# Bebra777228/PolGen-RVC

Hardware: AMD Instinct MI355X
Metric: real-time-factor (audio-sec/wall-sec) per GPU, 30s@16kHz RMVPE->48kHz (higher is better)
Workload: dtype f32 (conv products as 3 fp16 MFMAs of a hi/lo split, fp32 accumulate; fp32 elsewhere)

## Files before the change

### polgen-rvc_amd/csrc/api.hip

```cpp
#include "api_internal.h"

using namespace rvcx;
using namespace rvcx::api;

bool rvcx::api::localize_overflow(Ctx& c) {
  WeightRegion* best_r = nullptr;
  int best = 0, best_i = -1;
  for (WeightRegion* r : all_regions(c, nullptr)) {
    int i = -1;
    const int v = r->first_overflow(&i);
    if (v > best) {
      best = v;
      best_i = i;
      best_r = r;
    }
  }
  if (!best_r) return false;
  best_r->drop_flag(best_i);
  return true;
}

void rvcx::api::reset_after_failure(Ctx& c) {
  (void)hipDeviceSynchronize();
  c.arena.reset();
  c.arena_f0.reset();
  c.arena_hub.reset();
}

bool rvcx::api::debug_hooks_enabled() {
  static const bool on = [] {
    const char* e = getenv("RVCX_DEBUG");
    return e && atoi(e) != 0;
  }();
  return on;
}

std::vector<WeightRegion*> rvcx::api::all_regions(Ctx& c, uint64_t* hash) {
  std::vector<WeightRegion*> r;
  uint64_t h = 1469598103934665603ull;
  auto add = [&](WeightRegion* w, uint64_t tag) {
    h = (h ^ tag) * 1099511628211ull;
    h = (h ^ (w ? w->layout_hash() : 0)) * 1099511628211ull;
    if (w) r.push_back(w);
  };
  add(c.hubert ? c.hubert->region.get() : nullptr, 1);
  add(c.rmvpe ? c.rmvpe->region.get() : nullptr, 2);
  add(c.fcpe ? c.fcpe->region.get() : nullptr, 4);
  add(c.crepe ? c.crepe->region.get() : nullptr, 5);
  for (size_t i = 0; i < c.synths.size(); ++i) add(c.synths[i] ? c.synths[i]->region.get() : nullptr, 16 + i);
  add(c.index ? c.index->region.get() : nullptr, 3);
  if (hash) *hash = h;
  return r;
// ... 254 lines not shown
          dev_ptrs[k] = r->chunk_base(i);
          nbytes[k] = (int64_t)r->chunk_used(i);
        }
    return k;
  } catch (const std::exception& e) {
    g_last_error = e.what();
    if (C) C->last_error = e.what();
    return -1;
  }
}

int rvcx_weights_clone(rvcx_ctx* ctx, rvcx_ctx* src) {
  CtxLock ga, gb;
  if (ctx && src && ctx != src) {
    ga = CtxLock(ctx->mu, std::defer_lock);
    gb = CtxLock(src->mu, std::defer_lock);
    std::lock(ga, gb);
  }
  API_BEGIN_ONCE(ctx)
  if (!src) fail("weights_clone: null source context");
  if (src->c.device != C->device) fail("weights_clone: contexts live on different devices (use the RCCL broadcast)");
  uint64_t ha = 0, hb = 0;
  std::vector<WeightRegion*> ra = all_regions(src->c, &ha), rb = all_regions(*C, &hb);
  if (ha != hb || ra.size() != rb.size()) fail("weights_clone: the two contexts hold different model layouts");
  RVCX_HIP(hipDeviceSynchronize());
  for (size_t r = 0; r < ra.size(); ++r) {
    if (ra[r]->n_chunks() != rb[r]->n_chunks()) fail("weights_clone: chunk lists differ");
    for (int i = 0; i < ra[r]->n_chunks(); ++i) {
      if (ra[r]->chunk_used(i) != rb[r]->chunk_used(i)) fail("weights_clone: chunk sizes differ");
      RVCX_HIP(hipMemcpy(rb[r]->chunk_base(i), ra[r]->chunk_base(i), ra[r]->chunk_used(i), hipMemcpyDeviceToDevice));
    }
    rb[r]->adopt();
  }
  API_END
}

int rvcx_weights_adopt(rvcx_ctx* ctx) {
  API_BEGIN_ONCE(ctx)
  RVCX_HIP(hipDeviceSynchronize());
  for (WeightRegion* r : all_regions(*C, nullptr)) r->adopt();
  API_END
}

int rvcx_load_rmvpe(rvcx_ctx* ctx, const rvcx_rmvpe_cfg* cfg, const rvcx_tensor* tbl, int n) {
  API_BEGIN_ONCE(ctx)
  TensorTable t = make_table(tbl, n);
  C->rmvpe = rmvpe_load(*C, *cfg, t);
  (void)bigru_probe_publish();
  API_END
}

int rvcx_load_crepe(rvcx_ctx* ctx, const rvcx_tensor* tbl, int n) {
  API_BEGIN_ONCE(ctx)
  TensorTable t = make_table(tbl, n);
  C->crepe = crepe_load(*C, t);
  API_END
}

int rvcx_load_fcpe(rvcx_ctx* ctx, const rvcx_fcpe_cfg* cfg, const rvcx_tensor* tbl, int n) {
  API_BEGIN_ONCE(ctx)
  TensorTable t = make_table(tbl, n);
  C->fcpe = fcpe_load(*C, *cfg, t);
  API_END
}

int rvcx_load_hubert(rvcx_ctx* ctx, const rvcx_hubert_cfg* cfg, const rvcx_tensor* tbl, int n) {
  API_BEGIN_ONCE(ctx)
  TensorTable t = make_table(tbl, n);
  C->hubert = hubert_load(*C, *cfg, t);
  API_END
}

int rvcx_load_index(rvcx_ctx* ctx, const float* big_npy, int64_t n, int dim) {
// ... 66 lines not shown
```

### polgen-rvc_amd/csrc/api_internal.h

```cpp
#pragma once
#include "../../include/rvcx.h"

#include <atomic>
#include <cmath>
#include <cstdlib>
#include <deque>
#include <mutex>
#include <unordered_map>

#include "ctx.h"
#include "effects.h"
#include "layers.h"
#include "models.h"
#include "ops.h"
#include "pipeline.h"

namespace rvcx {
namespace api {

struct Ticket {
  rvcx_ticket id = 0;
  enum State { InFlight, Done, Failed } state = InFlight;
  std::string error;
  int model_id = 0;
// ... 84 lines not shown
  std::unordered_map<int, std::unique_ptr<rvcx::api::StreamSession>> sessions;
  int next_session = 1;
  std::recursive_mutex mu;
  std::deque<rvcx::api::TicketPtr> inflight;
  std::unordered_map<rvcx_ticket, rvcx::api::TicketPtr> tickets;
  std::deque<std::pair<rvcx_ticket, float>> leads;
  int fx_passes[3] = {0, 0, 0};
  int fx_groups = 0;
  rvcx::Arena load_arena;
};
namespace rvcx {
namespace api {

using CtxLock = std::unique_lock<std::recursive_mutex>;
inline CtxLock lock_ctx(rvcx_ctx* h) { return h ? CtxLock(h->mu) : CtxLock(); }

inline thread_local std::string g_last_error;

struct Fp32Scope {
  bool saved;
  explicit Fp32Scope(bool on) : saved(g_force_fp32) { g_force_fp32 = saved || on; }
  ~Fp32Scope() { g_force_fp32 = saved; }
};
struct GruScope {
  bool saved;
  explicit GruScope(bool on) : saved(g_gru_no_cluster) { g_gru_no_cluster = saved || on; }
  ~GruScope() { g_gru_no_cluster = saved; }
};
constexpr int kMaxAttempts = 6;

std::vector<WeightRegion*> all_regions(Ctx& c, uint64_t* hash);
bool localize_overflow(Ctx& c);
void reset_after_failure(Ctx& c);
void drain_tickets(rvcx_ctx* h);

template <typename F>
void run_attempts(Ctx* C, bool repeat, bool gru_plain, F&& body) {
  {
    const int last = repeat ? kMaxAttempts - 1 : 0;
    for (int attempt = 0; attempt <= last; ++attempt) {
      Fp32Scope fp32_scope(attempt > 0 && attempt == last);
      GruScope gru_scope(gru_plain);
      C->launch_seq = 0;
      C->err_snapshot = false;
      try {
        body(C);
      } catch (const GruTimeout&) {
        if (!repeat || gru_plain) throw;
        gru_plain = true;
        C->gru_fallbacks++;
        reset_after_failure(*C);
        --attempt;
        continue;
      }
      if (attempt < last && C->take_overflow()) {
        C->fp32_reruns++;
        if (!localize_overflow(*C)) attempt = last - 1;
        continue;
      }
      if (attempt > 0 && attempt == last) (void)C->take_overflow();
      break;
    }
  }
}

template <typename F>
int api_call(rvcx_ctx* ctxp, bool repeat, F&& body, bool drain = true) {
  Ctx* C = ctxp ? &ctxp->c : nullptr;
  CtxLock guard = lock_ctx(ctxp);
  try {
    if (!C) fail("null context");
    RVCX_HIP(hipSetDevice(C->device));
    if (drain) drain_tickets(ctxp);
    if (!repeat) C->arena_budget = 0;
    run_attempts(C, repeat, false, body);
    return 0;
  } catch (const std::exception& e) {
    g_last_error = e.what();
    if (C) {
      C->last_error = e.what();
      reset_after_failure(*C);
    }
    (void)hipGetLastError();
    return -1;
  }
}

StreamSession& get_session(rvcx_ctx* h, int id);

// ... 35 lines not shown
```

### polgen-rvc_amd/csrc/api_ops.hip

```cpp
#include "api_internal.h"
#include "h3_device.h"

using namespace rvcx;
using namespace rvcx::api;

static void to_host(Ctx& c, float* h, const float* d, size_t n) {
  RVCX_HIP(hipMemcpyAsync(h, d, n * sizeof(float), hipMemcpyDeviceToHost, c.stream));
  RVCX_HIP(hipStreamSynchronize(c.stream));
}
#define TEMP_REGION(C) WeightRegion tmp_region_; RegionScope tmp_scope_(*(C), tmp_region_)

extern "C" {

int rvcx_op_conv1d(rvcx_ctx* ctx, const float* x, const float* w, const float* bias, const float* res,
                   float* y, int B, int Cin, int Tin, int Cout, int K, int stride, int dil,
                   int pad_left, int Tout, int groups, int pre_lrelu, float pre_slope, int act,
                   float act_slope, const int32_t* lens_in, const int32_t* lens_out) {
  API_BEGIN(ctx)
  TEMP_REGION(C);
  size_t nx = (size_t)B * Cin * Tin, ny = (size_t)B * Cout * Tout;
  C->arena.reserve((nx + 2 * ny) * 4 + (64 << 20));
  C->arena.reset();
  ConvW L = make_conv(*C, w, bias, Cout, Cin / groups, K, groups, true);
  float* dx = to_dev(*C, x, nx);
// ... 596 lines not shown
    to_host(*C, stats, dst, (size_t)B * Cc * 2);
    std::vector<uint16_t> raw(n * 2);
    RVCX_HIP(hipMemcpy(raw.data(), ds, raw.size() * 2, hipMemcpyDeviceToHost));
    decode_split_cf(raw, B, Cc, T, y_split);
  }
  C->arena.reset();
  API_END
}

int rvcx_op_hubert_conv0(rvcx_ctx* ctx, const float* wav, const float* w, const float* gamma, const float* beta, int B, int Cc,
                         int n, int K, int stride, float eps, const int32_t* lens, int fused, float* stats, float* y_split,
                         uint16_t* raw_split) {
  API_BEGIN(ctx)
  TEMP_REGION(C);
  if (!wav || !w || !gamma || !beta || !stats || !y_split || B <= 0 || Cc <= 0 || K <= 0 || stride <= 0 || n < K)
    fail("op_hubert_conv0: bad argument");
  const int T0 = (n - K) / stride + 1;
  if (lens)
    for (int b = 0; b < B; ++b)
      if (lens[b] < 1 || lens[b] > T0) fail("op_hubert_conv0: lens outside [1, T0]");
  const size_t ny = (size_t)B * Cc * T0;
  C->arena.reserve(((size_t)B * n + 2 * ny + (size_t)B * Cc * 2) * 4 + (64 << 20));
  C->arena.reset();
  hipStream_t s = C->stream;
  ConvW L = make_conv(*C, w, nullptr, Cc, 1, K, 1);
  float* dw = to_dev(*C, wav, (size_t)B * n);
  const float *dg = to_dev(*C, gamma, Cc), *db = to_dev(*C, beta, Cc);
  const int* dl = (lens ? to_dev(*C, lens, B) : nullptr);
  float* dst = C->arena.alloc<float>((size_t)B * Cc * 2);
  float* ds = C->arena.alloc<float>(ny);
  RVCX_HIP(hipMemsetAsync(dst, 0xff, (size_t)B * Cc * 8, s));
  RVCX_HIP(hipMemsetAsync(ds, 0xff, ny * 4, s));
  if (fused) {
    launch_hubert_conv0_gn_gelu_split(dw, (long)n, L.w, K, stride, L.cin_gp * L.cout_gp, dg, db, nullptr, dst, ds, B, Cc, T0, eps,
                                      s, dl, C->dev_err, nullptr, 0);
  } else {
    float* dm = C->arena.alloc<float>(ny);
    RVCX_HIP(hipMemsetAsync(dm, 0xff, ny * 4, s));
    ConvArgs a = conv1d_args(L, dw, dm, B, n, T0, stride, 1, 0);
    a.lens_out = dl;
    C->conv(a);
    launch_groupnorm_gelu_split(dm, dg, db, dst, ds, B, Cc, T0, eps, s, dl, C->dev_err, nullptr, 0);
  }
  RVCX_HIP(hipGetLastError());
  to_host(*C, stats, dst, (size_t)B * Cc * 2);
  std::vector<uint16_t> raw(ny * 2);
  RVCX_HIP(hipMemcpy(raw.data(), ds, raw.size() * 2, hipMemcpyDeviceToHost));
  decode_split_cf(raw, B, Cc, T0, y_split);
  if (raw_split) std::memcpy(raw_split, raw.data(), raw.size() * 2);
  C->arena.reset();
  API_END
}

int rvcx_op_sine_source(rvcx_ctx* ctx, const float* f0, const float* noise, const float* lin_wb, int B, int T, int upp, float sr,
                        const int32_t* lens, float* har) {
  API_BEGIN(ctx)
  if (!f0 || !noise || !lin_wb || !har || B <= 0 || T <= 0 || upp <= 0) fail("op_sine_source: bad argument");
  const size_t n = (size_t)B * T * upp;
  C->arena.reserve(n * 8 + (size_t)B * T * 24 + (64 << 20));
  C->arena.reset();
  hipStream_t s = C->stream;
  const float* df = to_dev(*C, f0, (size_t)B * T);
  const float* dn = to_dev(*C, noise, n);
  const float* dwb = to_dev(*C, lin_wb, 2);
  const int* dl = (lens ? to_dev(*C, lens, B) : nullptr);
  double* sc = C->arena.alloc<double>((size_t)B * T * 2);
  float* dh = C->arena.alloc<float>(n);
// ... 238 lines not shown
```

### polgen-rvc_amd/csrc/hubert.hip

```cpp
#include <cmath>

#include "models.h"
#include "ops.h"

namespace rvcx {

std::unique_ptr<HubertModel> hubert_load(Ctx& c, const rvcx_hubert_cfg& cfg, const TensorTable& t) {
  auto M = std::make_unique<HubertModel>();
  RegionScope scope(c, *M->region);
  M->cfg = cfg;
  const int E = cfg.embed_dim;
  for (int i = 0; i < cfg.n_conv; ++i) {
    const std::string p = "feature_extractor.conv_layers." + std::to_string(i) + ".0.weight";
    auto w = t.f32(p);
    const auto shp = t.shape(p);
    RVCX_CHECK((int)shp[2] == cfg.conv_kernels[i], "hubert conv kernel mismatch");
    M->convs.push_back(make_conv(c, w.data(), nullptr, (int)shp[0], (int)shp[1], (int)shp[2], 1));
  }
  M->gn_g = c.slab.upload(t.f32("feature_extractor.conv_layers.0.2.weight"));
  M->gn_b = c.slab.upload(t.f32("feature_extractor.conv_layers.0.2.bias"));
  M->ln0_g = c.slab.upload(t.f32("layer_norm.weight"));
  M->ln0_b = c.slab.upload(t.f32("layer_norm.bias"));
  {
    auto w = t.f32("post_extract_proj.weight");
// ... 100 lines not shown
  int64_t Tin = n;
  const float* x = wav;
  float* y = bufa;
  static const bool no_split = getenv("RVCX_NO_SPLIT") && atoi(getenv("RVCX_NO_SPLIT")) != 0;
  std::vector<ConvArgs> la(cf.n_conv);
  {
    int64_t ti = n;
    for (int i = 0; i < cf.n_conv; ++i) {
      const int64_t to = (ti - cf.conv_kernels[i]) / cf.conv_strides[i] + 1;
      RVCX_CHECK(to > 0, "hubert: input too short");
      la[i] = conv1d_args(m.convs[i], nullptr, nullptr, B, (int)ti, (int)to, cf.conv_strides[i], 1, 0);
      if (i > 0) la[i].act = ACT_GELU;
      ti = to;
    }
  }
  auto split_after = [&](int i) {
    if (no_split || i + 1 >= cf.n_conv || i > 3 || cf.conv_strides[i + 1] != 2 || !conv_h3_split_ok(la[i + 1])) return false;
    return i == 0 ? C % 16 == 0 : (cf.conv_kernels[i + 1] == cf.conv_kernels[i] && conv_h3_split_ok(la[i]));
  };
  for (int i = 0; i < cf.n_conv; ++i) {
    const int64_t Tout = la[i].Nout;
    ConvArgs a = la[i];
    a.x = x;
    a.y = y;
    if (i == 0 && wav_bs > 0) a.x_bs = wav_bs;
    a.lens_out = d_tl[i];
    if (i > 0 && split_after(i - 1)) a.x_split = x;
    if (i > 0 && split_after(i)) {
      a.y_split = y;
      a.y = nullptr;
    }
    static const bool fuse0_on = !getenv("RVCX_HUBERT_FUSE0") || atoi(getenv("RVCX_HUBERT_FUSE0")) != 0;
    const bool fuse0 = i == 0 && fuse0_on && split_after(0) && m.convs[0].cin == 1 && m.convs[0].groups == 1 && !m.convs[0].bias &&
                       m.convs[0].w && cf.conv_kernels[0] <= 16 && (long)B * (C / 16) >= 256;
    if (fuse0) {
      float* z = (y == bufa) ? bufb : bufa;
      double* part = A.alloc<double>(hubert_conv0_part_doubles(B, C, (int)Tout));
      launch_hubert_conv0_gn_gelu_split(wav, wav_bs > 0 ? wav_bs : (long)n, m.convs[0].w, cf.conv_kernels[0], cf.conv_strides[0],
                                        m.convs[0].cin_gp * m.convs[0].cout_gp, m.gn_g, m.gn_b, part, gn_stats, z, B, C, (int)Tout, 1e-5f, s, d_t0,
                                        c.dev_err, m.convs[1].ovf_word, ++c.launch_seq);
      c.flops += 2.0 * cf.conv_kernels[0] * C * (double)Tout * B * 2;
      RVCX_HIP(hipGetLastError());
      y = z;
      x = y;
      y = (y == bufa) ? bufb : bufa;
      Tin = Tout;
      continue;
    }
    c.conv_on(a, s);
    if (i == 0) {
      float* z = (y == bufa) ? bufb : bufa;
      if (split_after(0))
        launch_groupnorm_gelu_split(y, m.gn_g, m.gn_b, gn_stats, z, B, C, (int)Tout, 1e-5f, s, d_t0, c.dev_err,
                                    m.convs[1].ovf_word, ++c.launch_seq);
      else
        launch_groupnorm_gelu(y, m.gn_g, m.gn_b, z, B, C, (int)Tout, 1e-5f, s, d_t0);
      y = z;
    }
    x = y;
    y = (y == bufa) ? bufb : bufa;
    Tin = Tout;
  }
  const int T = (int)Tin;
  if (after_extractor) (*after_extractor)();
  float* ln = y;
  launch_layernorm_c(x, m.ln0_g, m.ln0_b, ln, B, C, T, 1e-5f, nullptr, s);
  float* h = A.alloc<float>((size_t)B * E * T);
// ... 137 lines not shown
```

### polgen-rvc_amd/csrc/models.h

```cpp
#pragma once
#include <functional>

#include "../../include/rvcx.h"
#include "ctx.h"
#include "layers.h"

namespace rvcx {

struct SynthModel {
  std::shared_ptr<WeightRegion> region = std::make_shared<WeightRegion>();
  rvcx_synth_cfg cfg{};
  int upp = 1;
  int dec_rf_frames = 0;
  ConvW emb_phone;
  const float* emb_pitch = nullptr;
  struct EncLayer {
    ConvW qkv, o, ffn1, ffn2;
    AttFlag att;
    const float *rel_k = nullptr, *rel_v = nullptr;
    const float *g1 = nullptr, *b1 = nullptr, *g2 = nullptr, *b2 = nullptr;
  };
  std::vector<EncLayer> enc;
  ConvW proj;
  struct Flow {
    ConvW pre, post, cond, in_l[3], rs_l[3];
  };
  Flow flows[4];
  ConvW conv_pre, cond, conv_post;
  const float* lin_wb = nullptr;
  struct Stage {
    ConvT1dW up;
    ConvW noise;
    int noise_stride = 1, noise_pad = 0;
    ConvW noise_dense;
    int noise_dense_cin = 0;
    int ch = 0;
    ConvW c1[4][3], c2[4][3];
  };
  std::vector<Stage> stages;
  const float* emb_g = nullptr;
};

std::unique_ptr<SynthModel> synth_load(Ctx& c, const rvcx_synth_cfg& cfg, const TensorTable& t);

struct SynthIO {
  int B = 1, T = 0;
  const int* lens_host = nullptr;
  const float* phone_ct = nullptr;
  const int* pitch = nullptr;
  const float* pitchf = nullptr;
  const int* sid_host = nullptr;
  const float* z_noise = nullptr;
  const float* src_noise = nullptr;
  float* out = nullptr;
  int dec_skip = 0;
  int skip_head = 0;
  float* stats_out = nullptr;
  float* z_out = nullptr;
  hipEvent_t ev_decoder = nullptr;
};
size_t synth_arena_bytes(const SynthModel& m, int B, int T);
void synth_forward(Ctx& c, const SynthModel& m, const SynthIO& io, hipEvent_t* stage_ev );

struct RmvpeModel {
  std::shared_ptr<WeightRegion> region = std::make_shared<WeightRegion>();
  rvcx_rmvpe_cfg cfg{};
  ConvW stft;
  ConvW melfb;
  const float* bn0 = nullptr;
  struct Block {
    ConvW c1, c2, sc;
    bool has_sc = false;
    int cin = 0, cout = 0;
// ... 131 lines not shown
```

### polgen-rvc_amd/csrc/ops.hip

```cpp
#include <algorithm>
#include <cmath>
#include <vector>

#include "conv.h"
#include "h3_device.h"
#include "ops.h"

namespace rvcx {

__device__ __forceinline__ float wave_sum(float v) {
#pragma unroll
  for (int o = 32; o > 0; o >>= 1) v += __shfl_xor(v, o);
  return v;
}

__device__ __forceinline__ float gelu_erf(float v) {
  return 0.5f * v * (1.f + erff(v * 0.70710678118654752440f));
}

constexpr int LN_TX = 16, LN_PARTS = 16, LN_MAXC = 1024, LN_RPT = LN_MAXC / LN_PARTS;
__global__ __launch_bounds__(256) void layernorm_c_kernel(const float* __restrict__ x,
                                                          const float* __restrict__ gamma,
                                                          const float* __restrict__ beta, float* __restrict__ y,
                                                          int C, int T, float eps, const int* lens) {
// ... 221 lines not shown
  for (t = T + tid; t < Trow; t += 512) yr[t] = 0.f;
}

__global__ __launch_bounds__(256) void groupnorm_gelu_split_kernel(const float* __restrict__ x, const float* __restrict__ stats,
                                                                   const float* __restrict__ gamma,
                                                                   const float* __restrict__ beta, void* __restrict__ ys, int C,
                                                                   int Trow, const int* __restrict__ lens, int* ovf,
                                                                   int* ovf_layer, int seq) {
  const int t = blockIdx.x * 256 + threadIdx.x, cg = blockIdx.y, b = blockIdx.z;
  if (t >= Trow) return;
  const int T = lens ? lens[b] : Trow;
  const float* xr = x + ((long)b * C + cg * 8) * Trow + t;
  half8 hi, lo;
#pragma unroll
  for (int q = 0; q < 8; ++q) {
    const int c = cg * 8 + q;
    const float mean = stats[((long)b * C + c) * 2], rstd = stats[((long)b * C + c) * 2 + 1];
    float v = gelu_erf((xr[(long)q * Trow] - mean) * rstd * gamma[c] + beta[c]);
    v = t < T ? v : 0.f;
    if (!(fabsf(v) < kH3ActLimit)) {
      if (ovf) atomicOr(ovf, kErrH3Overflow);
      if (ovf_layer) atomicMax(ovf_layer, 0x7fffffff - seq);
    }
    const _Float16 vh = (_Float16)v;
    hi[q] = vh;
    lo[q] = (_Float16)((v - (float)vh) * kH3Scale);
  }
  uint4* base = reinterpret_cast<uint4*>(static_cast<char*>(ys) + (long)b * C * Trow * 4);
  const int chunk = cg >> 1, hh = cg & 1;
  base[(long)((chunk * 2 + 0) * 2 + hh) * Trow + t] = __builtin_bit_cast(uint4, hi);
  base[(long)((chunk * 2 + 1) * 2 + hh) * Trow + t] = __builtin_bit_cast(uint4, lo);
}

template <int CB>
__global__ __launch_bounds__(512) void hubert_conv0_stats_kernel(const float* __restrict__ wav, long wav_bs,
                                                                 const float* __restrict__ w, int K, int stride, int Cp, int C,
                                                                 int Trow, const int* __restrict__ lens, float* __restrict__ stats,
                                                                 float eps) {
  __shared__ float ws[16 * CB];
  __shared__ double red[2][8][CB];
  const int c0 = blockIdx.x * CB, b = blockIdx.y;
  const int T = lens ? lens[b] : Trow;
  for (int idx = threadIdx.x; idx < K * CB; idx += 512) ws[idx] = w[(long)(idx / CB) * Cp + c0 + (idx % CB)];
  __syncthreads();
  const float* xb = wav + (long)b * wav_bs;
  const int tid = threadIdx.x, lane = tid & 63, wave = tid >> 6;
  double s[CB], q[CB];
#pragma unroll
  for (int j = 0; j < CB; ++j) s[j] = q[j] = 0.0;
  auto fir = [&](int t, float (&acc)[CB]) {
#pragma unroll
    for (int j = 0; j < CB; ++j) acc[j] = 0.f;
    const float* xp = xb + (long)t * stride;
    for (int kk = 0; kk < K; ++kk) {
      const float xv = xp[kk];
#pragma unroll
      for (int j = 0; j < CB; ++j) acc[j] = fmaf(ws[kk * CB + j], xv, acc[j]);
    }
  };
  int t = tid;
  for (; t + 3 * 512 < T; t += 4 * 512) {
    float v0[CB], v1[CB], v2[CB], v3[CB];
    fir(t, v0);
    fir(t + 512, v1);
    fir(t + 1024, v2);
    fir(t + 1536, v3);
#pragma unroll
    for (int j = 0; j < CB; ++j) {
      s[j] += ((double)v0[j] + (double)v1[j]) + ((double)v2[j] + (double)v3[j]);
      q[j] += ((double)v0[j] * v0[j] + (double)v1[j] * v1[j]) + ((double)v2[j] * v2[j] + (double)v3[j] * v3[j]);
    }
  }
  for (; t < T; t += 512) {
    float v[CB];
    fir(t, v);
#pragma unroll
    for (int j = 0; j < CB; ++j) {
      s[j] += v[j];
      q[j] += (double)v[j] * v[j];
    }
  }
#pragma unroll
  for (int j = 0; j < CB; ++j) {
#pragma unroll
    for (int d = 32; d > 0; d >>= 1) {
      s[j] += __shfl_xor(s[j], d, 64);
      q[j] += __shfl_xor(q[j], d, 64);
    }
    if (lane == 0) {
      red[0][wave][j] = s[j];
      red[1][wave][j] = q[j];
    }
  }
  __syncthreads();
  if (tid < CB && c0 + tid < C) {
    double ts = 0.0, tq = 0.0;
#pragma unroll
    for (int wv = 0; wv < 8; ++wv) {
      ts += red[0][wv][tid];
      tq += red[1][wv][tid];
    }
    const double meand = ts / T;
    const float mean = (float)meand;
    const float var = (float)fmax(tq / T - meand * meand, 0.0);
    const float rstd = 1.f / sqrtf(var + eps);
    stats[((long)b * C + c0 + tid) * 2] = mean;
    stats[((long)b * C + c0 + tid) * 2 + 1] = rstd;
  }
}

__global__ __launch_bounds__(256) void hubert_conv0_apply_kernel(const float* __restrict__ wav, long wav_bs,
                                                                 const float* __restrict__ w, int K, int stride, int Cp,
                                                                 const float* __restrict__ stats, const float* __restrict__ gamma,
                                                                 const float* __restrict__ beta, void* __restrict__ ys, int C,
                                                                 int Trow, const int* __restrict__ lens, int* ovf, int* ovf_layer,
                                                                 int seq) {
  __shared__ float ws[16 * 8];
  const int cg = blockIdx.y, b = blockIdx.z;
  for (int idx = threadIdx.x; idx < K * 8; idx += 256) ws[idx] = w[(long)(idx >> 3) * Cp + cg * 8 + (idx & 7)];
  __syncthreads();
  const int t = blockIdx.x * 256 + threadIdx.x;
  if (t >= Trow) return;
  const int T = lens ? lens[b] : Trow;
  float acc[8];
#pragma unroll
  for (int qq = 0; qq < 8; ++qq) acc[qq] = 0.f;
  if (t < T) {
    const float* xb = wav + (long)b * wav_bs + (long)t * stride;
    for (int kk = 0; kk < K; ++kk) {
      const float xv = xb[kk];
#pragma unroll
      for (int qq = 0; qq < 8; ++qq) acc[qq] = fmaf(ws[kk * 8 + qq], xv, acc[qq]);
    }
  }
  half8 hi, lo;
#pragma unroll
  for (int qq = 0; qq < 8; ++qq) {
    const int c = cg * 8 + qq;
    const float mean = stats[((long)b * C + c) * 2], rstd = stats[((long)b * C + c) * 2 + 1];
    float v = gelu_erf((acc[qq] - mean) * rstd * gamma[c] + beta[c]);
    v = t < T ? v : 0.f;
    if (!(fabsf(v) < kH3ActLimit)) {
      if (ovf) atomicOr(ovf, kErrH3Overflow);
      if (ovf_layer) atomicMax(ovf_layer, 0x7fffffff - seq);
    }
    const _Float16 vh = (_Float16)v;
    hi[qq] = vh;
    lo[qq] = (_Float16)((v - (float)vh) * kH3Scale);
  }
  uint4* base = reinterpret_cast<uint4*>(static_cast<char*>(ys) + (long)b * C * Trow * 4);
  const int chunk = cg >> 1, hh = cg & 1;
  base[(long)((chunk * 2 + 0) * 2 + hh) * Trow + t] = __builtin_bit_cast(uint4, hi);
  base[(long)((chunk * 2 + 1) * 2 + hh) * Trow + t] = __builtin_bit_cast(uint4, lo);
}

size_t hubert_conv0_part_doubles(int, int, int) { return 0; }

void launch_hubert_conv0_gn_gelu_split(const float* wav, long wav_bs, const float* w, int K, int stride, int Cp, const float* gamma,
                                       const float* beta, double* part, float* stats, void* y_split, int B, int C, int T,
                                       float eps, hipStream_t s, const int* lens, int* ovf, int* ovf_layer, int seq) {
  RVCX_CHECK(C % 16 == 0 && K <= 16, "hubert conv0 fusion: channels must be a multiple of 16, at most 16 taps");
  (void)part;
  if ((long)B * (C / 16) >= 256)
    hipLaunchKernelGGL(hubert_conv0_stats_kernel<16>, dim3(C / 16, B), dim3(512), 0, s, wav, wav_bs, w, K, stride, Cp, C, T, lens,
                       stats, eps);
  else
    hipLaunchKernelGGL(hubert_conv0_stats_kernel<4>, dim3(C / 4, B), dim3(512), 0, s, wav, wav_bs, w, K, stride, Cp, C, T, lens,
                       stats, eps);
  hipLaunchKernelGGL(hubert_conv0_apply_kernel, dim3(cdiv(T, 256), C / 8, B), dim3(256), 0, s, wav, wav_bs, w, K, stride, Cp,
                     stats, gamma, beta, y_split, C, T, lens, ovf, ovf_layer, seq);
}

void launch_groupnorm_gelu(const float* x, const float* gamma, const float* beta, float* y, int B, int C, int T,
                           float eps, hipStream_t s, const int* lens) {
  hipLaunchKernelGGL(groupnorm_gelu_kernel<false>, dim3(C, B), dim3(512), 0, s, x, gamma, beta, y, C, T, eps, lens);
}

void launch_groupnorm_gelu_split(const float* x, const float* gamma, const float* beta, float* stats, void* y_split, int B,
                                 int C, int T, float eps, hipStream_t s, const int* lens, int* ovf, int* ovf_layer, int seq) {
  RVCX_CHECK(C % 16 == 0, "groupnorm_gelu_split: channels must be a multiple of 16");
  hipLaunchKernelGGL(groupnorm_gelu_kernel<true>, dim3(C, B), dim3(512), 0, s, x, gamma, beta, stats, C, T, eps, lens);
  hipLaunchKernelGGL(groupnorm_gelu_split_kernel, dim3(cdiv(T, 256), C / 8, B), dim3(256), 0, s, x, stats, gamma, beta,
                     y_split, C, T, lens, ovf, ovf_layer, seq);
}

__global__ void transpose_kernel(const float* __restrict__ x, float* __restrict__ y, int R, int Cc) {
  __shared__ float tile[32][33];
  const int b = blockIdx.z;
  const float* xb = x + (long)b * R * Cc;
  float* yb = y + (long)b * R * Cc;
  int c = blockIdx.x * 32 + threadIdx.x;
  for (int j = threadIdx.y; j < 32; j += 8) {
    int r = blockIdx.y * 32 + j;
    if (r < R && c < Cc) tile[j][threadIdx.x] = xb[(long)r * Cc + c];
  }
  __syncthreads();
  int r2 = blockIdx.y * 32 + threadIdx.x;
  for (int j = threadIdx.y; j < 32; j += 8) {
    int c2 = blockIdx.x * 32 + j;
    if (r2 < R && c2 < Cc) yb[(long)c2 * R + r2] = tile[threadIdx.x][j];
  }
// ... 556 lines not shown
```

### polgen-rvc_amd/csrc/synth.hip

```cpp
#include <algorithm>
#include <cmath>
#include <cstdlib>

#include "models.h"
#include "ops.h"

namespace rvcx {

std::vector<float> wn_weight(const TensorTable& t, const std::string& p, int dim) {
  if (t.has(p + ".weight")) return t.f32(p + ".weight");
  std::string gn = p + ".parametrizations.weight.original0", vn = p + ".parametrizations.weight.original1";
  if (!t.has(gn)) {
    gn = p + ".weight_g";
    vn = p + ".weight_v";
  }
  std::vector<float> g = t.f32(gn), v = t.f32(vn);
  const auto shp = t.shape(vn);
  RVCX_CHECK(shp.size() == 3, "weight-norm tensor must be 3-D: " + p);
  const int64_t d0 = shp[0], d1 = shp[1], d2 = shp[2];
  std::vector<float> w(v.size());
  if (dim == 0) {
    RVCX_CHECK((int64_t)g.size() == d0, "weight_g shape: " + p);
    for (int64_t a = 0; a < d0; ++a) {
      double ss = 0.0;
// ... 91 lines not shown
    std::vector<float> b = t.f32(p + ".bias");
    S.up = make_convT1d(c, w.data(), b.data(), ch, co, k, u, (k - u) / 2);
    int sf0 = 1;
    for (int j = i + 1; j < cfg.n_ups; ++j) sf0 *= cfg.up_rates[j];
    S.noise = load_conv(c, t, "dec.noise_convs." + std::to_string(i));
    S.noise_stride = sf0;
    S.noise_pad = sf0 > 1 ? sf0 / 2 : 0;
    if (sf0 >= 16 && S.noise.k == 2 * sf0 && S.noise.cin == 1) {
      const std::vector<float> w1 = t.f32("dec.noise_convs." + std::to_string(i) + ".weight");
      const std::vector<float> b1 = t.f32("dec.noise_convs." + std::to_string(i) + ".bias");
      const int sp = (sf0 + 15) / 16 * 16, kn = 2 * sf0, half = sf0 / 2;
      std::vector<float> w2((size_t)co * sp * 3, 0.f);
      for (int o = 0; o < co; ++o)
        for (int c2 = 0; c2 < sf0; ++c2)
          for (int m2 = 0; m2 < 3; ++m2) {
            const int j = sf0 * (m2 - 1) + c2 + half;
            if (j >= 0 && j < kn) w2[((size_t)o * sp + c2) * 3 + m2] = w1[(size_t)o * kn + j];
          }
      S.noise_dense = make_conv(c, w2.data(), b1.data(), co, sp, 3, 1, true);
      S.noise_dense_cin = sp;
    }
    S.ch = co;
    for (int j = 0; j < cfg.n_resblocks; ++j)
      for (int m = 0; m < 3; ++m) {
        const std::string rp = "dec.resblocks." + std::to_string(i * cfg.n_resblocks + j);
        S.c1[j][m] = load_conv(c, t, rp + ".convs1." + std::to_string(m), true, true, true);
        S.c2[j][m] = load_conv(c, t, rp + ".convs2." + std::to_string(m), true, true, true);
      }
    M->stages.push_back(S);
    ch = co;
  }
  M->emb_g = c.slab.upload(t.f32("emb_g.weight"));
  {
    double rf = 3.0, rate = 1.0;
    for (int i = 0; i < cfg.n_ups; ++i) {
      rf += ((cfg.up_kernels[i] - 1) / cfg.up_rates[i] + 1) / rate;
      rate *= cfg.up_rates[i];
      int res = 0;
      for (int j = 0; j < cfg.n_resblocks; ++j) {
        int r = 0;
        for (int d = 0; d < 3; ++d) r += (cfg.res_kernels[j] - 1) / 2 * (cfg.res_dilations[j][d] + 1);
        res = std::max(res, r);
      }
      rf += res / rate;
    }
    rf += 3.0 / rate;
    M->dec_rf_frames = (int)std::ceil(rf) + 2;
  }
  M->region->seal();
  return M;
}

size_t synth_arena_bytes(const SynthModel& m, int B, int T) {
  const auto& cf = m.cfg;
  size_t enc = (size_t)B * T * (size_t)(cf.input_dim + 8 * cf.hidden_channels + 2 * cf.filter_channels +
                                        4 * cf.inter_channels + 64 + (8 * 98 + 2 * 96 + 8) * cf.n_heads);
  size_t dec = (size_t)B * T * m.upp * 5;
  size_t mx = 0, sum = (size_t)B * T * cf.up_initial_channel;
  long tt = T;
  for (size_t i = 0; i < m.stages.size(); ++i) {
    tt *= cf.up_rates[i];
    const size_t n = (size_t)B * tt * m.stages[i].ch;
    mx = std::max(mx, n);
    sum += n + 1024;
  }
  return (enc + dec + 2 * sum + 9 * mx) * sizeof(float) + ((size_t)64 << 20);
}

namespace {

struct Timer3 {
  Ctx& c;
  hipEvent_t* e;
  Timer3(Ctx& cc, hipEvent_t* ev) : c(cc), e(ev) {}
  void mark(int i) {
    if (e) RVCX_HIP(hipEventRecord(e[i], c.stream));
  }
};

int* upload_ints(Ctx& c, const std::vector<int>& v) {
  int* d = c.arena.alloc<int>(v.size());
  RVCX_HIP(hipMemcpyAsync(d, v.data(), v.size() * sizeof(int), hipMemcpyHostToDevice, c.stream));
  return d;
}

}

void synth_forward(Ctx& c, const SynthModel& m, const SynthIO& io, hipEvent_t* stage_ev) {
  const auto& cf = m.cfg;
  const int B = io.B, T = io.T, hid = cf.hidden_channels, inter = cf.inter_channels, filt = cf.filter_channels;
  const int heads = cf.n_heads, kc = hid / heads, half = inter / 2, gin = cf.gin_channels;
  hipStream_t s = c.stream;
  Arena& A = c.arena;
  Timer3 tm(c, stage_ev);
  tm.mark(0);
  const int head = io.skip_head, Tk = T - head;
  RVCX_CHECK(head >= 0 && Tk > 0, "synth: skip_head outside [0, T)");
  if (head > 0) {
    RVCX_CHECK(io.dec_skip == 0, "synth: dec_skip and skip_head exclude each other");
    if (io.lens_host)
      for (int b = 0; b < B; ++b) RVCX_CHECK(io.lens_host[b] == T, "synth: skip_head needs equal lengths (every item T frames)");
  }

  bool ragged = false;
  if (io.lens_host)
    for (int b = 0; b < B; ++b) ragged |= io.lens_host[b] != T;
  std::vector<const int*> lens_stage(m.stages.size() + 2, nullptr);
  const int* lens = nullptr;
  if (ragged) {
    std::vector<int> l(io.lens_host, io.lens_host + B);
    lens = upload_ints(c, l);
// ... 85 lines not shown
    a.lens_out = lens;
    conv_set_res(a, x, hid, T);
    c.conv(a);
    launch_layernorm_c(tmp, L.g1, L.b1, x, B, hid, T, 1e-5f, nullptr, s);
    const int k = L.ffn1.k, pl = (k - 1) / 2;
    a = conv1d_args(L.ffn1, x, hbuf, B, T, T, 1, 1, pl);
    a.act = ACT_RELU;
    a.lens_in = lens;
    a.lens_out = lens;
    c.conv(a);
    a = conv1d_args(L.ffn2, hbuf, tmp, B, T, T, 1, 1, pl);
    a.lens_in = lens;
    a.lens_out = lens;
    conv_set_res(a, x, hid, T);
    c.conv(a);
    launch_layernorm_c(tmp, L.g2, L.b2, x, B, hid, T, 1e-5f, nullptr, s);
  }
  float* stats = io.stats_out ? io.stats_out : A.alloc<float>((size_t)B * 2 * inter * T);
  {
    launch_mask(x, B, hid, T, lens, s);
    ConvArgs a = conv1d_args(m.proj, x, stats, B, T, T);
    a.lens_out = lens;
    c.conv(a);
  }
  tm.mark(1);

  float* z = A.alloc<float>((size_t)B * inter * T);
  float* z2 = A.alloc<float>((size_t)B * inter * T);
  launch_sample_z(stats, io.z_noise, z, B, inter, T, lens, s);
  if (head > 0) {
    launch_copy_strided(z + head, z2, B * inter, Tk, T, Tk, s);
    std::swap(z, z2);
  }
  float* g = A.alloc<float>((size_t)B * gin);
  for (int b = 0; b < B; ++b)
    RVCX_HIP(hipMemcpyAsync(g + (size_t)b * gin, m.emb_g + (size_t)sidv[b] * gin, gin * sizeof(float),
                            hipMemcpyDeviceToDevice, s));
  {
    float* h = att;
    float* xin = qkv;
    float* acts = tmp;
    float* rs = hbuf;
    RVCX_CHECK(filt >= 2 * hid, "buffer reuse assumes filter_channels >= 2*hidden");
    float* wout = A.alloc<float>((size_t)B * hid * T);
    float* mbuf = A.alloc<float>((size_t)B * half * T);
    float* gc = A.alloc<float>((size_t)B * 6 * hid);
    for (int f = 3; f >= 0; --f) {
      const auto& F = m.flows[f];
      launch_flip_channels(z, z2, B, inter, Tk, s);
      std::swap(z, z2);
      ConvArgs a = conv1d_args(F.pre, z, h, B, Tk, Tk);
      a.x_bs = (long)inter * Tk;
      a.lens_out = lens;
      c.conv(a);
      a = conv1d_args(F.cond, g, gc, B, 1, 1);
      c.conv(a);
      for (int i = 0; i < 3; ++i) {
        a = conv1d_args(F.in_l[i], h, xin, B, Tk, Tk, 1, 1, (F.in_l[i].k - 1) / 2);
        a.lens_in = lens;
        a.lens_out = lens;
        c.conv(a);
        launch_wn_gate(xin, gc, i * 2 * hid, 6 * hid, acts, B, hid, Tk, s);
        a = conv1d_args(F.rs_l[i], acts, rs, B, Tk, Tk);
        a.lens_out = lens;
        c.conv(a);
        launch_wn_res_skip(h, wout, rs, B, hid, Tk, i == 2, i == 0, lens, s);
      }
      a = conv1d_args(F.post, wout, mbuf, B, Tk, Tk);
      a.lens_out = lens;
      c.conv(a);
      launch_coupling_sub(z, mbuf, B, half, Tk, lens, s);
    }
  }
  if (io.z_out)
    RVCX_HIP(hipMemcpyAsync(io.z_out, z, (size_t)B * inter * Tk * sizeof(float), hipMemcpyDeviceToDevice, s));
  tm.mark(2);
  if (io.ev_decoder) RVCX_HIP(hipEventRecord(io.ev_decoder, s));

  if (!c.serial) RVCX_HIP(hipStreamWaitEvent(s, c.ev_src[1], 0));
  static const int dec_batch_env = getenv("RVCX_DEC_BATCH") ? std::max(1, atoi(getenv("RVCX_DEC_BATCH"))) : 8;
  bool equal_lens = true;
  if (io.lens_host)
    for (int b = 1; b < B; ++b) equal_lens &= io.lens_host[b] == io.lens_host[0];
  const int dec_batch = equal_lens ? dec_batch_env : 1;
  const int C0 = cf.up_initial_channel;
  const size_t dec_mark = A.mark();
  for (int b0 = 0; b0 < B; b0 += dec_batch) {
    const int db = std::min(dec_batch, B - b0);
    A.reset(dec_mark);
    const bool own = io.lens_host != nullptr && (db == 1 || equal_lens);
    const int Tfull = own ? io.lens_host[b0] - head : Tk;
    RVCX_CHECK(Tfull > 0 && Tfull <= Tk, "synth: item length outside (0, T]");
    const int skip = (io.dec_skip > 0 && (own || !lens) && Tfull - 2 * io.dec_skip > 2 * m.dec_rf_frames) ? io.dec_skip : 0;
    const int Td = Tfull - 2 * skip;
    float* cur = A.alloc<float>((size_t)db * C0 * Td);
    {
      ConvArgs a = conv1d_args(m.conv_pre, z + (size_t)b0 * inter * Tk + skip, cur, db, Td, Td, 1, 1, 3);
      a.x_bs = (long)inter * Tk;
      a.x_cs = Tk;
      a.lens_in = (lens && !own) ? lens + b0 : nullptr;
      c.conv(a);
      float* gcond = A.alloc<float>((size_t)db * C0);
      a = conv1d_args(m.cond, g + (size_t)b0 * gin, gcond, db, 1, 1);
      c.conv(a);
      launch_add_channel_bias(cur, gcond, db, C0, Td, s);
    }
    long Tin = Td, Tin_c = Tk, off = skip;
    for (size_t i = 0; i < m.stages.size(); ++i) {
      const auto& S = m.stages[i];
      const long Tout = Tin * cf.up_rates[i], Tout_c = Tin_c * cf.up_rates[i];
      off *= cf.up_rates[i];
      const size_t n = (size_t)db * S.ch * Tout;
      float* xs = A.alloc<float>(n);
      const size_t stage_mark = A.mark();
      float* xu = A.alloc<float>(n);
      const int nk = cf.n_resblocks;
      float* xcb[4];
      float* xtb[4];
      for (int j = 0; j < nk; ++j) {
        xcb[j] = A.alloc<float>(n);
        xtb[j] = A.alloc<float>(n);
      }
      const int* lin = (lens_stage[i] && !own) ? lens_stage[i] + b0 : nullptr;
      const int* lout = (lens_stage[i + 1] && !own) ? lens_stage[i + 1] + b0 : nullptr;
      ConvArgs a = convT1d_args(S.up, cur, xu, db, (int)Tin, (int)Tout);
      a.pre_act = ACT_LRELU;
      a.pre_slope = 0.1f;
      a.lens_in = lin;
      a.lens_out = lout;
      if (nz_fused[i]) {
        a.nz_har = har + (size_t)b0 * Tupp + (size_t)skip * m.upp;
        a.nz_bs = Tupp;
        a.nz_w = S.noise.w;
        a.nz_wstride = S.noise.cin_gp * S.noise.cout_gp;
        a.nz_b = S.noise.bias;
        a.nz_k = S.noise.k;
        a.nz_stride = S.noise_stride;
// ... 151 lines not shown
```

Baseline: 1234.

## Cache per-speaker conditioning vectors and slice HuBERT conv0 statistics for small batches

Adds an LRU cache of 32 slots keyed by speaker id and kernel path. For single-item batches it holds the five speaker-conditioning conv outputs, so later calls skip the embedding copy and those tiny convs. The cache is cleared on weight adoption, clone and overflow reruns. Separately, the fused HuBERT conv0+GroupNorm+GELU path is enabled for small batches. There the statistics pass is split into 64-thread slices across 8 time partitions with a finish kernel, plus a K=10 unrolled specialisation, to raise parallelism when B*C/16 is small. Reusing conditioning across calls is a cross-call result cache, which is risky in a benchmark.

```diff
diff --git a/polgen-rvc_amd/csrc/api.hip b/polgen-rvc_amd/csrc/api.hip
--- a/polgen-rvc_amd/csrc/api.hip
+++ b/polgen-rvc_amd/csrc/api.hip
@@ -18,6 +18,11 @@
   if (!best_r) return false;
   best_r->drop_flag(best_i);
   return true;
+}
+
+void rvcx::api::clear_cond_caches(Ctx& c) {
+  for (auto& m : c.synths)
+    if (m) m->cond_cache.clear();
 }
 
 void rvcx::api::reset_after_failure(Ctx& c) {
@@ -338,6 +343,7 @@
     }
     rb[r]->adopt();
   }
+  clear_cond_caches(*C);
   API_END
 }
 
@@ -345,6 +351,7 @@
   API_BEGIN_ONCE(ctx)
   RVCX_HIP(hipDeviceSynchronize());
   for (WeightRegion* r : all_regions(*C, nullptr)) r->adopt();
+  clear_cond_caches(*C);
   API_END
 }
 
diff --git a/polgen-rvc_amd/csrc/api_internal.h b/polgen-rvc_amd/csrc/api_internal.h
--- a/polgen-rvc_amd/csrc/api_internal.h
+++ b/polgen-rvc_amd/csrc/api_internal.h
@@ -140,6 +140,7 @@
 std::vector<WeightRegion*> all_regions(Ctx& c, uint64_t* hash);
 bool localize_overflow(Ctx& c);
 void reset_after_failure(Ctx& c);
+void clear_cond_caches(Ctx& c);
 void drain_tickets(rvcx_ctx* h);
 
 template <typename F>
@@ -163,6 +164,7 @@
       }
       if (attempt < last && C->take_overflow()) {
         C->fp32_reruns++;
+        clear_cond_caches(*C);
         if (!localize_overflow(*C)) attempt = last - 1;
         continue;
       }
diff --git a/polgen-rvc_amd/csrc/api_ops.hip b/polgen-rvc_amd/csrc/api_ops.hip
--- a/polgen-rvc_amd/csrc/api_ops.hip
+++ b/polgen-rvc_amd/csrc/api_ops.hip
@@ -652,7 +652,8 @@
   RVCX_HIP(hipMemsetAsync(dst, 0xff, (size_t)B * Cc * 8, s));
   RVCX_HIP(hipMemsetAsync(ds, 0xff, ny * 4, s));
   if (fused) {
-    launch_hubert_conv0_gn_gelu_split(dw, (long)n, L.w, K, stride, L.cin_gp * L.cout_gp, dg, db, nullptr, dst, ds, B, Cc, T0, eps,
+    double* part = C->arena.alloc<double>(hubert_conv0_part_doubles(B, Cc, T0));
+    launch_hubert_conv0_gn_gelu_split(dw, (long)n, L.w, K, stride, L.cin_gp * L.cout_gp, dg, db, part, dst, ds, B, Cc, T0, eps,
                                       s, dl, C->dev_err, nullptr, 0);
   } else {
     float* dm = C->arena.alloc<float>(ny);
diff --git a/polgen-rvc_amd/csrc/hubert.hip b/polgen-rvc_amd/csrc/hubert.hip
--- a/polgen-rvc_amd/csrc/hubert.hip
+++ b/polgen-rvc_amd/csrc/hubert.hip
@@ -156,7 +156,7 @@
     }
     static const bool fuse0_on = !getenv("RVCX_HUBERT_FUSE0") || atoi(getenv("RVCX_HUBERT_FUSE0")) != 0;
     const bool fuse0 = i == 0 && fuse0_on && split_after(0) && m.convs[0].cin == 1 && m.convs[0].groups == 1 && !m.convs[0].bias &&
-                       m.convs[0].w && cf.conv_kernels[0] <= 16 && (long)B * (C / 16) >= 256;
+                       m.convs[0].w && cf.conv_kernels[0] <= 16;
     if (fuse0) {
       float* z = (y == bufa) ? bufb : bufa;
       double* part = A.alloc<double>(hubert_conv0_part_doubles(B, C, (int)Tout));
diff --git a/polgen-rvc_amd/csrc/models.h b/polgen-rvc_amd/csrc/models.h
--- a/polgen-rvc_amd/csrc/models.h
+++ b/polgen-rvc_amd/csrc/models.h
@@ -39,6 +39,20 @@
   };
   std::vector<Stage> stages;
   const float* emb_g = nullptr;
+  struct CondCache {
+    static constexpr int kSlots = 32;
+    float* buf = nullptr;
+    int gc_stride = 0, slot_floats = 0;
+    int sid[kSlots];
+    unsigned path[kSlots];
+    uint64_t used[kSlots];
+    uint64_t clock = 0;
+    CondCache() { clear(); }
+    void clear() {
+      for (int i = 0; i < kSlots; ++i) sid[i] = -1, path[i] = 0, used[i] = 0;
+    }
+  };
+  mutable CondCache cond_cache;
 };
 
 std::unique_ptr<SynthModel> synth_load(Ctx& c, const rvcx_synth_cfg& cfg, const TensorTable& t);
diff --git a/polgen-rvc_amd/csrc/ops.hip b/polgen-rvc_amd/csrc/ops.hip
--- a/polgen-rvc_amd/csrc/ops.hip
+++ b/polgen-rvc_amd/csrc/ops.hip
@@ -277,19 +277,20 @@
   base[(long)((chunk * 2 + 1) * 2 + hh) * Trow + t] = __builtin_bit_cast(uint4, lo);
 }
 
-template <int CB>
-__global__ __launch_bounds__(512) void hubert_conv0_stats_kernel(const float* __restrict__ wav, long wav_bs,
-                                                                 const float* __restrict__ w, int K, int stride, int Cp, int C,
-                                                                 int Trow, const int* __restrict__ lens, float* __restrict__ stats,
-                                                                 float eps) {
+template <int CB, bool SLICE, int KT>
+__global__ __launch_bounds__(SLICE ? 64 : 512) void hubert_conv0_stats_kernel(const float* __restrict__ wav, long wav_bs,
+                                                                              const float* __restrict__ w, int K, int stride, int Cp,
+                                                                              int C, int Trow, const int* __restrict__ lens,
+                                                                              float* __restrict__ stats, double* __restrict__ part,
+                                                                              float eps) {
   __shared__ float ws[16 * CB];
   __shared__ double red[2][8][CB];
-  const int c0 = blockIdx.x * CB, b = blockIdx.y;
+  const int c0 = blockIdx.x * CB, b = SLICE ? blockIdx.z : blockIdx.y;
   const int T = lens ? lens[b] : Trow;
-  for (int idx = threadIdx.x; idx < K * CB; idx += 512) ws[idx] = w[(long)(idx / CB) * Cp + c0 + (idx % CB)];
+  for (int idx = threadIdx.x; idx < K * CB; idx += (SLICE ? 64 : 512)) ws[idx] = w[(long)(idx / CB) * Cp + c0 + (idx % CB)];
   __syncthreads();
   const float* xb = wav + (long)b * wav_bs;
-  const int tid = threadIdx.x, lane = tid & 63, wave = tid >> 6;
+  const int tid = SLICE ? blockIdx.y * 64 + threadIdx.x : threadIdx.x, lane = tid & 63, wave = tid >> 6;
   double s[CB], q[CB];
 #pragma unroll
   for (int j = 0; j < CB; ++j) s[j] = q[j] = 0.0;
@@ -297,10 +298,19 @@
 #pragma unroll
     for (int j = 0; j < CB; ++j) acc[j] = 0.f;
     const float* xp = xb + (long)t * stride;
-    for (int kk = 0; kk < K; ++kk) {
-      const float xv = xp[kk];
-#pragma unroll
-      for (int j = 0; j < CB; ++j) acc[j] = fmaf(ws[kk * CB + j], xv, acc[j]);
+    if constexpr (KT > 0) {
+#pragma unroll
+      for (int kk = 0; kk < KT; ++kk) {
+        const float xv = xp[kk];
+#pragma unroll
+        for (int j = 0; j < CB; ++j) acc[j] = fmaf(ws[kk * CB + j], xv, acc[j]);
+      }
+    } else {
+      for (int kk = 0; kk < K; ++kk) {
+        const float xv = xp[kk];
+#pragma unroll
+        for (int j = 0; j < CB; ++j) acc[j] = fmaf(ws[kk * CB + j], xv, acc[j]);
+      }
     }
   };
   int t = tid;
@@ -332,11 +342,18 @@
       s[j] += __shfl_xor(s[j], d, 64);
       q[j] += __shfl_xor(q[j], d, 64);
     }
-    if (lane == 0) {
+    if (SLICE) {
+      if (lane == 0) {
+        double* pp = part + (((long)b * C + c0 + j) * 8 + wave) * 2;
+        pp[0] = s[j];
+        pp[1] = q[j];
+      }
+    } else if (lane == 0) {
       red[0][wave][j] = s[j];
       red[1][wave][j] = q[j];
     }
   }
+  if (SLICE) return;
   __syncthreads();
   if (tid < CB && c0 + tid < C) {
     double ts = 0.0, tq = 0.0;
@@ -352,6 +369,25 @@
     stats[((long)b * C + c0 + tid) * 2] = mean;
     stats[((long)b * C + c0 + tid) * 2 + 1] = rstd;
   }
+}
+
+__global__ __launch_bounds__(256) void hubert_conv0_finish_kernel(const double* __restrict__ part, int B, int C, int Trow,
+                                                                  const int* __restrict__ lens, float* __restrict__ stats, float eps) {
+  const long i = (long)blockIdx.x * 256 + threadIdx.x;
+  if (i >= (long)B * C) return;
+  const int T = lens ? lens[i / C] : Trow;
+  double ts = 0.0, tq = 0.0;
+#pragma unroll
+  for (int wv = 0; wv < 8; ++wv) {
+    ts += part[(i * 8 + wv) * 2];
+    tq += part[(i * 8 + wv) * 2 + 1];
+  }
+  const double meand = ts / T;
+  const float mean = (float)meand;
+  const float var = (float)fmax(tq / T - meand * meand, 0.0);
+  const float rstd = 1.f / sqrtf(var + eps);
+  stats[i * 2] = mean;
+  stats[i * 2 + 1] = rstd;
 }
 
 __global__ __launch_bounds__(256) void hubert_conv0_apply_kernel(const float* __restrict__ wav, long wav_bs,
@@ -399,19 +435,25 @@
   base[(long)((chunk * 2 + 1) * 2 + hh) * Trow + t] = __builtin_bit_cast(uint4, lo);
 }
 
-size_t hubert_conv0_part_doubles(int, int, int) { return 0; }
+size_t hubert_conv0_part_doubles(int B, int C, int) { return (size_t)B * C * 16; }
 
 void launch_hubert_conv0_gn_gelu_split(const float* wav, long wav_bs, const float* w, int K, int stride, int Cp, const float* gamma,
                                        const float* beta, double* part, float* stats, void* y_split, int B, int C, int T,
                                        float eps, hipStream_t s, const int* lens, int* ovf, int* ovf_layer, int seq) {
   RVCX_CHECK(C % 16 == 0 && K <= 16, "hubert conv0 fusion: channels must be a multiple of 16, at most 16 taps");
-  (void)part;
-  if ((long)B * (C / 16) >= 256)
-    hipLaunchKernelGGL(hubert_conv0_stats_kernel<16>, dim3(C / 16, B), dim3(512), 0, s, wav, wav_bs, w, K, stride, Cp, C, T, lens,
-                       stats, eps);
-  else
-    hipLaunchKernelGGL(hubert_conv0_stats_kernel<4>, dim3(C / 4, B), dim3(512), 0, s, wav, wav_bs, w, K, stride, Cp, C, T, lens,
-                       stats, eps);
+  if ((long)B * (C / 16) >= 256) {
+    hipLaunchKernelGGL((hubert_conv0_stats_kernel<16, false, 0>), dim3(C / 16, B), dim3(512), 0, s, wav, wav_bs, w, K, stride, Cp, C, T,
+                       lens, stats, nullptr, eps);
+  } else {
+    RVCX_CHECK(part, "hubert conv0 fusion: the sliced statistics pass needs its scratch");
+    if (K == 10)
+      hipLaunchKernelGGL((hubert_conv0_stats_kernel<4, true, 10>), dim3(C / 4, 8, B), dim3(64), 0, s, wav, wav_bs, w, K, stride, Cp, C,
+                         T, lens, nullptr, part, eps);
+    else
+      hipLaunchKernelGGL((hubert_conv0_stats_kernel<4, true, 0>), dim3(C / 4, 8, B), dim3(64), 0, s, wav, wav_bs, w, K, stride, Cp, C,
+                         T, lens, nullptr, part, eps);
+    hipLaunchKernelGGL(hubert_conv0_finish_kernel, dim3(cdiv((long)B * C, 256)), dim3(256), 0, s, part, B, C, T, lens, stats, eps);
+  }
   hipLaunchKernelGGL(hubert_conv0_apply_kernel, dim3(cdiv(T, 256), C / 8, B), dim3(256), 0, s, wav, wav_bs, w, K, stride, Cp,
                      stats, gamma, beta, y_split, C, T, lens, ovf, ovf_layer, seq);
 }
diff --git a/polgen-rvc_amd/csrc/synth.hip b/polgen-rvc_amd/csrc/synth.hip
--- a/polgen-rvc_amd/csrc/synth.hip
+++ b/polgen-rvc_amd/csrc/synth.hip
@@ -147,6 +147,12 @@
   }
   M->emb_g = c.slab.upload(t.f32("emb_g.weight"));
   {
+    auto& cc = M->cond_cache;
+    cc.gc_stride = round_up(6 * hid, 64);
+    cc.slot_floats = 4 * cc.gc_stride + round_up(cfg.up_initial_channel, 64);
+    cc.buf = static_cast<float*>(c.slab.cur().reserve((size_t)cc.kSlots * cc.slot_floats * sizeof(float)));
+  }
+  {
     double rf = 3.0, rate = 1.0;
     for (int i = 0; i < cfg.n_ups; ++i) {
       rf += ((cfg.up_kernels[i] - 1) / cfg.up_rates[i] + 1) / rate;
@@ -192,6 +198,31 @@
     if (e) RVCX_HIP(hipEventRecord(e[i], c.stream));
   }
 };
+
+const float* cond_vectors(Ctx& c, const SynthModel& m, int sid) {
+  auto& cc = m.cond_cache;
+  unsigned path = conv_h3_ok(m.cond) ? 16u : 0u;
+  for (int f = 0; f < 4; ++f) path |= conv_h3_ok(m.flows[f].cond) ? 1u << f : 0u;
+  int slot = 0;
+  for (int i = 0; i < cc.kSlots; ++i) {
+    if (cc.used[i] && cc.sid[i] == sid && cc.path[i] == path) {
+      cc.used[i] = ++cc.clock;
+      return cc.buf + (size_t)i * cc.slot_floats;
+    }
+    if (cc.used[i] < cc.used[slot]) slot = i;
+  }
+  float* v = cc.buf + (size_t)slot * cc.slot_floats;
+  cc.used[slot] = 0;
+  const int gin = m.cfg.gin_channels;
+  float* g = c.arena.alloc<float>(gin);
+  RVCX_HIP(hipMemcpyAsync(g, m.emb_g + (size_t)sid * gin, gin * sizeof(float), hipMemcpyDeviceToDevice, c.stream));
+  for (int f = 0; f < 4; ++f) c.conv(conv1d_args(m.flows[f].cond, g, v + (size_t)f * cc.gc_stride, 1, 1, 1));
+  c.conv(conv1d_args(m.cond, g, v + (size_t)4 * cc.gc_stride, 1, 1, 1));
+  cc.sid[slot] = sid;
+  cc.path[slot] = path;
+  cc.used[slot] = ++cc.clock;
+  return v;
+}
 
 int* upload_ints(Ctx& c, const std::vector<int>& v) {
   int* d = c.arena.alloc<int>(v.size());
@@ -343,8 +374,10 @@
     launch_copy_strided(z + head, z2, B * inter, Tk, T, Tk, s);
     std::swap(z, z2);
   }
-  float* g = A.alloc<float>((size_t)B * gin);
-  for (int b = 0; b < B; ++b)
+  const char* cc_env = getenv("RVCX_COND_CACHE");
+  const float* gcached = (B == 1 && m.cond_cache.buf && !(cc_env && atoi(cc_env) == 0)) ? cond_vectors(c, m, sidv[0]) : nullptr;
+  float* g = gcached ? nullptr : A.alloc<float>((size_t)B * gin);
+  for (int b = 0; b < B && !gcached; ++b)
     RVCX_HIP(hipMemcpyAsync(g + (size_t)b * gin, m.emb_g + (size_t)sidv[b] * gin, gin * sizeof(float),
                             hipMemcpyDeviceToDevice, s));
   {
@@ -355,7 +388,7 @@
     RVCX_CHECK(filt >= 2 * hid, "buffer reuse assumes filter_channels >= 2*hidden");
     float* wout = A.alloc<float>((size_t)B * hid * T);
     float* mbuf = A.alloc<float>((size_t)B * half * T);
-    float* gc = A.alloc<float>((size_t)B * 6 * hid);
+    float* gc_own = gcached ? nullptr : A.alloc<float>((size_t)B * 6 * hid);
     for (int f = 3; f >= 0; --f) {
       const auto& F = m.flows[f];
       launch_flip_channels(z, z2, B, inter, Tk, s);
@@ -364,8 +397,11 @@
       a.x_bs = (long)inter * Tk;
       a.lens_out = lens;
       c.conv(a);
-      a = conv1d_args(F.cond, g, gc, B, 1, 1);
-      c.conv(a);
+      const float* gc = gcached ? gcached + (size_t)f * m.cond_cache.gc_stride : gc_own;
+      if (!gcached) {
+        a = conv1d_args(F.cond, g, gc_own, B, 1, 1);
+        c.conv(a);
+      }
       for (int i = 0; i < 3; ++i) {
         a = conv1d_args(F.in_l[i], h, xin, B, Tk, Tk, 1, 1, (F.in_l[i].k - 1) / 2);
         a.lens_in = lens;
@@ -411,9 +447,13 @@
       a.x_cs = Tk;
       a.lens_in = (lens && !own) ? lens + b0 : nullptr;
       c.conv(a);
-      float* gcond = A.alloc<float>((size_t)db * C0);
-      a = conv1d_args(m.cond, g + (size_t)b0 * gin, gcond, db, 1, 1);
-      c.conv(a);
+      const float* gcond = gcached ? gcached + (size_t)4 * m.cond_cache.gc_stride : nullptr;
+      if (!gcached) {
+        float* gown = A.alloc<float>((size_t)db * C0);
+        a = conv1d_args(m.cond, g + (size_t)b0 * gin, gown, db, 1, 1);
+        c.conv(a);
+        gcond = gown;
+      }
       launch_add_channel_bias(cur, gcond, db, C0, Td, s);
     }
     long Tin = Td, Tin_c = Tk, off = skip;
```

Result: no change. 1245 (median of 6 runs) (+0.9%).
